# LTLA/batchelor

Hardware: AMD Instinct MI355X
Metric: cells/sec corrected (reducedMNN engine, 50 PCs) (higher is better)
Workload: dtype fp16 MFMA candidate pass (f32 accumulate) + FP64 exact re-rank; 1 GPU; config3: 8 synthetic Gaussian batches x 100000 cells x 50 PCs, k=20, merge.order=1..8, inputs resident in HBM; parallelism=single GPU, exact_fallback_queries=1050

## Files before the change

### batchelor_amd/csrc/abi.hip

```cpp
#include <algorithm>
#include <chrono>
#include <climits>
#include <cstddef>
#include <cmath>
#include <cstdlib>
#include <cstring>
#include <functional>
#include <limits>
#include <memory>
#include <thread>
#include <vector>

#include "bmx_common.hpp"
#include "bmx_ops.hpp"
#include "engine.hpp"
#include "host_xfer.hpp"
#include "mnn_correct.hpp"
#include "rccl_dyn.hpp"
#include "resident_batches.hpp"

struct bmx_engine {
    std::unique_ptr<bmx::Engine> impl;
};
struct bmx_mnn_result {
// ... 140 lines not shown
        }
    });
}

void bmx_trim_caches(void) {
    bmx::DevBlockCache::release_global();
    bmx::StreamPool::release_all();
}

int64_t bmx_last_knn_exact_fallbacks(void) { return g_last_fallbacks; }

void bmx_set_force_exact_knn(int32_t on) { g_force_exact = on; }

int32_t bmx_dev_set(const char* name, int32_t value) {
    if (!name) return BMX_ERR_ARG;
    bmx::DevKnobs& k = bmx::dev_knobs();
    const std::string n(name);
    if (n == "knn_tier") k.knn_tier = value;
    else if (n == "sample") k.sample = value;
    else if (n == "split_c") k.split_c = value;
    else if (n == "force_c") k.force_c = value;
    else if (n == "no_margin") k.no_margin = value;
    else if (n == "asv_fast") k.asv_fast = value;
    else if (n == "asv_cap") k.asv_cap = value;
    else if (n == "sample_split") k.sample_split = value;
    else if (n == "lk_seed") k.lk_seed = value;
    else if (n == "asv_modes") k.asv_modes = value;
    else if (n == "asv_sync") k.asv_sync = value;
    else if (n == "tau_replay") k.tau_replay = value;
    else if (n == "exchange_always") k.exchange_always = value;
    else if (n == "refine_wave") k.refine_wave = value;
    else if (n == "asv_wide") k.asv_wide = value;
    else if (n == "asv_chunk") k.asv_chunk = value;
    else if (n == "reset") k = bmx::DevKnobs();
    else {
        g_last_error = "bmx_dev_set: unknown knob '" + n + "'";
        return BMX_ERR_ARG;
    }
    return BMX_OK;
}

int32_t bmx_dev_get(const char* name, int64_t* value) {
    if (!name || !value) return BMX_ERR_ARG;
    return guarded([&] {
        const std::string n(name);
        unsigned long long t[8];
        if (n == "asv_literal_cells" || n == "asv_fallback_cells" || n == "asv_tiled_cells") {
            bmx::asv_tally_read(t, false);
            *value = (int64_t)t[n == "asv_literal_cells" ? 0 : (n == "asv_fallback_cells" ? 1 : 2)];
        } else if (n == "asv_ticks_stream" || n == "asv_ticks_wait" || n == "asv_ticks_cells") {
            bmx::asv_ticks_read(t);
            *value = (int64_t)t[n == "asv_ticks_stream" ? 0 : (n == "asv_ticks_wait" ? 1 : 2)];
        } else if (n == "asv_ticks_literal" || n == "asv_ticks_chains" || n == "asv_literal_addends" || n == "asv_chain_tiles") {
            bmx::asv_ticks_read(t);
            *value = (int64_t)t[n == "asv_ticks_literal" ? 4 : (n == "asv_ticks_chains" ? 5 : (n == "asv_literal_addends" ? 6 : 7))];
        } else if (n == "delta_gene_tile" || n == "delta_pair_chunk") {
            *value = n == "delta_gene_tile" ? bmx::DELTA_GENE_TILE : bmx::DELTA_PAIR_CHUNK;
        } else if (n == "asv_tally_reset") {
            bmx::asv_tally_read(t, true);
            *value = 0;
        } else {
            throw bmx::Error(BMX_ERR_ARG, "bmx_dev_get: unknown counter '" + n + "'");
        }
    });
}

int32_t bmx_dev_get_bytes(const char* name, void* dst, int64_t n) {
    if (!name || (n > 0 && !dst) || n < 0) return BMX_ERR_ARG;
    return guarded([&] {
        if (std::string(name) != "asv_modes") throw bmx::Error(BMX_ERR_ARG, std::string("bmx_dev_get_bytes: unknown array '") + name + "'");
        bmx::asv_modes_read(static_cast<unsigned char*>(dst), (size_t)n);
    });
}

int32_t bmx_dev_host_copy(void* dst, const void* src, int64_t bytes) {
    if (bytes < 0 || (bytes > 0 && (!dst || !src))) return BMX_ERR_ARG;
    bmx::host_parallel_memcpy(dst, src, (size_t)bytes);
    return BMX_OK;
}

void bmx_shard_range(int64_t n, int32_t rank, int32_t world, int64_t* begin, int64_t* end) {
    bmx::bmx_shard_range_impl(n, rank, world, begin, end);
}

int64_t bmx_shard_gather_bytes(int64_t n, int32_t world, int64_t bytes_per_row) {
    return bmx::bmx_shard_rows_per_rank(n, world) * bytes_per_row;
}

int32_t bmx_query_knn(const double* X, int32_t nx, const double* query, int32_t nq, int32_t d, int32_t k,
                      int32_t* index, double* distance) {
    return guarded([&] {
        if (nx < 0 || nq < 0 || d <= 0 || k < 0) throw bmx::Error(BMX_ERR_ARG, "queryKNN: negative dimension");
        if (k > nx) throw bmx::Error(BMX_ERR_ARG, "queryKNN: 'k' exceeds the number of points in 'X'");
        if (nq == 0 || k == 0) return;
        bmx::Engine& e = prim(d);
        bmx::CacheScope cache_scope(e.cache());
        hipStream_t s = e.stream();
        bmx::DevBuf<double> t1, t2, dX, dQ, dD;
        bmx::DevBuf<int32_t> dI, dIc;
        const double* px = upload_rm(t1, dX, X, nx, d, s);
        const double* pq = upload_rm(t2, dQ, query, nq, d, s);
        int32_t* pi = dI.reserve((size_t)nq * k);
        double* pd = dD.reserve((size_t)nq * k);
        e.knn(px, nullptr, nx, pq, nullptr, nq, k, pi, pd);
        const size_t nres = (size_t)nq * k;
        if (nres >= ((size_t)1 << 22)) {
            g_last_fallbacks = e.knn_ws_.last_exact;
            if (index) {
                int32_t* pc = dIc.reserve(nres);
                hipLaunchKernelGGL(idx_to_r_layout, dim3((unsigned)((nq + 31) / 32), (unsigned)((k + 31) / 32)), dim3(32, 8), 0, s,
                                   (const int32_t*)pi, nq, k, pc);
// ... 678 lines not shown
```

### batchelor_amd/csrc/bmx_common.hpp

```cpp
#pragma once
#include <hip/hip_runtime.h>

#include <atomic>
#include <cstdint>
#include <cstdio>
#include <map>
#include <mutex>
#include <stdexcept>
#include <string>
#include <vector>

#include "../../include/batchelor_mi355x.h"

namespace bmx {

struct Error : std::runtime_error {
    int code;
    Error(int c, const std::string& m) : std::runtime_error(m), code(c) {}
};

#define BMX_HIP(expr)                                                                                   \
    do {                                                                                                \
        hipError_t e_ = (expr);                                                                         \
        if (e_ != hipSuccess)                                                                           \
            throw bmx::Error(BMX_ERR_HIP, std::string(#expr) + " failed: " + hipGetErrorString(e_));    \
    } while (0)

#define BMX_LAUNCH_CHECK() BMX_HIP(hipGetLastError())

struct WatchdogTimeout : Error {
    explicit WatchdogTimeout(const std::string& m) : Error(BMX_ERR_HIP, m) {}
};
void guarded_stream_sync(hipStream_t stream, double budget_s);

#ifndef BMX_KS1
#define BMX_KS1 32
#endif

struct DevKnobs {
    int knn_tier = 0;
    int sample = -1;
    int split_c = 0;
    int force_c = 0;
    int no_margin = 0;
    int asv_fast = 0;
    int asv_cap = -1;
    int asv_modes = 0;
    int asv_sync = 0;
    int tau_replay = 0;
    int lk_seed = 1;
    int sample_split = -1;
    int exchange_always = 0;
    int refine_wave = 0;
    int asv_wide = 0;
    int asv_chunk = 0;
};
DevKnobs& dev_knobs();
bool debug_prints();
bool debug_timings();

inline int cdiv(int64_t a, int64_t b) { return (int)((a + b - 1) / b); }
inline int64_t round_up(int64_t a, int64_t b) { return (a + b - 1) / b * b; }

struct DevBlockCache {
    struct Block {
        void* p;
        size_t bytes;
        int device;
    };
    std::vector<Block> blocks;
    bool leak = false;
    DevBlockCache() = default;
    DevBlockCache(const DevBlockCache&) = delete;
    DevBlockCache& operator=(const DevBlockCache&) = delete;
    struct GlobalPool {
        std::mutex mu;
        std::vector<Block> blocks;
        size_t total = 0;
    };
    static GlobalPool& global() {
        static GlobalPool* g = new GlobalPool();
        return *g;
    }
    ~DevBlockCache() {
        GlobalPool& g = global();
        if (!leak) {
            std::lock_guard<std::mutex> lk(g.mu);
// ... 185 lines not shown
            DevBlockCache* c = DevBlockCache::current();
            if (void* q = c ? c->take(want * sizeof(T), &got) : nullptr) {
                p = static_cast<T*>(q);
                cap = got / sizeof(T);
            } else {
                ++dev_malloc_calls();
                hipError_t e = hipMalloc((void**)&p, want * sizeof(T));
                if (e == hipErrorOutOfMemory) {
                    (void)hipGetLastError();
                    DevBlockCache::release_global();
                    e = hipMalloc((void**)&p, want * sizeof(T));
                }
                if (e != hipSuccess) {
                    p = nullptr;
                    throw bmx::Error(BMX_ERR_HIP, std::string("hipMalloc failed: ") + hipGetErrorString(e));
                }
                cap = want;
            }
        }
        return p;
    }
};

struct KnnWorkspace {
    DevBuf<float> pq, pr;
    DevBuf<double> qn2, rn2, mean, red;
    DevBuf<int32_t> cand;
    DevBuf<float> tau;
    DevBuf<float> cand_v;
    DevBuf<uint32_t> tau_g;
    DevBuf<float> margin;
    std::vector<DevBuf<uint32_t>> tau_rec;
    size_t replay_idx = 0;
    DevBuf<float> samp_lists;
    DevBuf<uint32_t> tau_seed;
    bool slots_clean = false;
    DevBuf<unsigned long long> maxslots;
    DevBuf<int32_t> flagged_t[2], sub_rows[2], sub_idx[2];
    DevBuf<int32_t> lk_rows, lk_idx;
    DevBuf<double> lk_d2;
    bool dist_squared = false;
    DevBuf<double> lk_kth;
    DevBuf<float> lk_seed;
    DevBuf<double> flag_bound_t[2], sub_dist[2];
    DevBuf<double> drow;
    DevBuf<double> xd;
    DevBuf<int32_t> xcnt, xi, slow;
    static constexpr int OPT_CAP = 256;
    bool optimistic = false;
    bool xcnt_clear = false;
    DevBuf<int32_t> opt_state;
    int32_t* opt_state_ptr(hipStream_t s) {
        if (!opt_state.p) {
            opt_state.reserve(8);
            BMX_HIP(hipMemsetAsync(opt_state.p, 0, 8 * sizeof(int32_t), s));
        }
        return opt_state.p;
    }
    int force_exact = 0;
    double wd_budget_s = 0.0;
    void sync(hipStream_t s) const { guarded_stream_sync(s, wd_budget_s); }
    int64_t* pinned_words() {
        if (!pin_) pin_ = static_cast<int64_t*>(pinned_small_take());
        return pin_;
    }
    static constexpr size_t kPinnedSmall = (size_t)64 << 10;
// ... 40 lines not shown
        if (event_tag.size() <= events_used) event_tag.resize(events_used + 1);
        event_tag[events_used] = tag;
        if (events_used == events.size()) {
            hipEvent_t a, b;
            BMX_HIP(hipEventCreate(&a));
            BMX_HIP(hipEventCreate(&b));
            events.emplace_back(a, b);
        }
        return events[events_used++];
    }
    ~KnnWorkspace() {
        if (abandon) return;
        pinned_small_give(pin_);
        for (auto& e : events) {
            (void)hipEventDestroy(e.first);
            (void)hipEventDestroy(e.second);
        }
    }
};

struct Bf16Launch {
    const uint16_t* pq;
    const uint16_t* pr;
    int nqb, first_begin, range_len, nranges, r_limit, out_chunk0, out_nchunks;
    uint32_t* tau_g;
    int sample;
    int32_t* cand;
    float* cand_v;
    float* tau;
    int n_full = 0;
    const float* margin = nullptr;
    int k = 0;
    const uint32_t* tau_seed = nullptr;
};
int bf16_pick_ns(int d);
int bf16_ncons(int NS, int KS);
void bf16_prep(hipStream_t stream, const double* X, const int32_t* rows, int n, int n_pad, int d, int NS,
               const double* mean, int is_query, uint16_t* P, double* n2, unsigned long long* maxbits,
               unsigned long long* slots);
bool bf16_launch(hipStream_t stream, KnnWorkspace& ws, int NS, int KS, const Bf16Launch& L);
int f16_rows_per_slot(int NS, int KS);

void knn_device(hipStream_t stream, KnnWorkspace& ws, const double* X, const int32_t* ref_rows, int nr,
                const double* Q, const int32_t* q_rows, int nq, int d, int k, int32_t* idx_out, double* dist_out,
                int q_begin, int q_end, const float* seed_d2 = nullptr, const double* centre = nullptr,
                double* kth_out = nullptr);

}
```

### batchelor_amd/csrc/knn.hip

```cpp
#include "bmx_common.hpp"
#include "knn_select.hpp"

#include <algorithm>
#include <atomic>
#include <chrono>
#include <cmath>
#include <cstdio>
#include <cstdlib>
#include <thread>

namespace bmx {

int f16_pick_ns(int d, int KS);
void f16_prep_all(hipStream_t stream, const double* X, const int32_t* rrows, int nr, int nr_pad, const double* Q,
                  const int32_t* qrows, int nq, int nq_pad, int d, int NS, const double* mean, uint16_t* Pr, uint16_t* Pq,
                  double* rn2, double* qn2, unsigned long long* maxbits, unsigned long long* slots, int32_t* flagged0,
                  float* margin, const sel::PassEps& pe, const float* seed_d2, uint32_t* tau_seed, uint32_t* tau_init);
bool f16_launch(hipStream_t stream, KnnWorkspace& ws, int NS, int KS, const Bf16Launch& L);
void f16_sample_merge(hipStream_t stream, const float* lists, int nranges, int KS, int nq, int k, const float* margin,
                      uint32_t* tau_g);

namespace {

using namespace sel;

constexpr int MAX_CHUNKS = 8;

__global__ void colsum_partial(const double* __restrict__ X, const int32_t* __restrict__ rows, int n, int d,
                               int rows_per_block, int stride, double* __restrict__ partial) {
    __shared__ double sm[4][64];
    const int c0 = threadIdx.x & 63, rl = threadIdx.x >> 6;
    const int r0 = blockIdx.x * rows_per_block;
    const int r1 = min(n, r0 + rows_per_block);
    for (int cb = 0; cb < d; cb += 64) {
        const int c = cb + c0;
        double s = 0.0;
        if (c < d)
            for (int r = r0 + rl; r < r1; r += 4) {
                const int64_t rs = (int64_t)r * stride;
                const int64_t row = rows ? rows[rs] : rs;
                s += X[row * d + c];
            }
        sm[rl][c0] = s;
        __syncthreads();
        if (rl == 0 && c < d) partial[(int64_t)blockIdx.x * d + c] = (sm[0][c0] + sm[1][c0]) + (sm[2][c0] + sm[3][c0]);
        __syncthreads();
    }
}

__global__ void colsum_final(const double* __restrict__ partial, int nblocks, int d, double scale,
                             double* __restrict__ out) {
    const int c = blockIdx.x * blockDim.x + threadIdx.x;
    if (c >= d) return;
    double s = 0.0;
    for (int b = 0; b < nblocks; ++b) s += partial[(int64_t)b * d + c];
    out[c] = s * scale;
}


// ... 841 lines not shown

int candidate_tiers(int d, int k, int nr, Tier out[2]) {
    const int only = dev_knobs().knn_tier;
    int n = 0;
    if (k > 36) return 0;
    const int KS1 = k <= 20 ? BMX_KS1 : 48, KS2 = k <= 20 ? 24 : 40;
    const int ns1 = f16_pick_ns(d, KS1);
    if (ns1 && nr > 2 * KS1 && (only == 0 || only == 1)) out[n++] = Tier{1, ns1, KS1};
    const int ns2 = bf16_pick_ns(d);
    if (ns2 && !(KS2 == 40 && ns2 > 16) && nr > 2 * KS2 && (only == 0 || only == 2)) out[n++] = Tier{2, ns2, KS2};
    return n;
}

void candidate_pass(hipStream_t stream, KnnWorkspace& ws, const Tier& T, const double* X, const int32_t* ref_rows, int nr,
                    const double* Qs, const int32_t* qrs, int nq, int d, int k, int32_t* io, double* dout,
                    int32_t* flagged, double* flag_bound, const float* seed_d2, const double* centre, double* kth_out) {
    const int NS = T.NS, KS = T.KS;
    ws.last_variant = T.id == 1 ? 3 : 2;
    const int unit = T.id == 1 ? 256 : 32 * bf16_ncons(NS, KS);
    const int nq_pad = (int)round_up(nq, unit);
    const int nqb = nq_pad / unit;

    const bool no_margin_knob = dev_knobs().no_margin != 0;
    int S_auto = nr >= 32768 ? 4096 : 0;
    if (T.id == 1 && nr >= 4096) S_auto = std::max(1024, std::min(nr / 4, NS <= 4 ? 24576 : 12288));
    if (seed_d2 && T.id == 1) S_auto = std::min(S_auto, BMX_SEEDED_SAMPLE);
    int S = (int)round_up(dev_knobs().sample >= 0 ? dev_knobs().sample : S_auto, T.id == 1 ? f16_rows_per_slot(NS, KS) : 64);
    int CS = 1;
    if (T.id == 1 && S > 0 && nqb < 128 && dev_knobs().sample_split != 0 && !no_margin_knob) {
        const int rs = f16_rows_per_slot(NS, KS);
        CS = std::max(1, std::min({256 / std::max(nqb, 1), 8, S / (8 * rs)}));
        if (dev_knobs().sample_split > 0) CS = std::max(1, std::min({dev_knobs().sample_split, S / rs, 512 / KS}));
    }
    int C = 1, n_full = 0;
    {
        const int a = nqb / 256, b = nqb % 256;
        n_full = a * 256;
        if (b > 0) {
            double best = 1e30;
            for (int c = 1; c <= MAX_CHUNKS - 1; ++c) {
                if (c > 1 && nr / c < 2048) break;
                const double tailc = std::ceil((double)b * c / 256.0) / c * (1.0 + 0.105 * std::log((double)c));
                if (tailc < best - 1e-9) {
                    best = tailc;
                    C = c;
                }
            }
        }
    }
    if (dev_knobs().split_c > 0) C = std::max(1, dev_knobs().split_c);
    if (dev_knobs().force_c > 0) {
        C = std::max(1, std::min(MAX_CHUNKS - 1, dev_knobs().force_c));
        n_full = 0;
    }
    const int rmul = T.id == 1 ? f16_rows_per_slot(NS, KS) : 32;
    const int chunk_len = (int)round_up(cdiv(nr, C), rmul);
    C = std::max(1, cdiv(nr, chunk_len));
    const int nr_pad = chunk_len * C;
    const int nchunks = C;
    S = std::min(S, nr_pad / rmul * rmul);
    if (debug_prints())
        fprintf(stderr, "[bmx] knn tier %d: nq=%d nr=%d d=%d NS=%d KS=%d S=%d C=%d chunk=%d full-range blocks=%d of %d\n", T.id,
                nq, nr, d, NS, KS, S, C, chunk_len, C > 1 ? n_full : nqb, nqb);

    const int KPw = 8 * NS;
    float* pq = ws.pq.reserve((size_t)nq_pad * KPw);
    float* pr = ws.pr.reserve((size_t)(nr_pad + 256) * KPw);
    double* qn2 = ws.qn2.reserve(nq_pad);
    double* rn2 = ws.rn2.reserve(nr_pad);
    double* mean = ws.mean.reserve((size_t)d + 2);
    unsigned long long* maxbits = reinterpret_cast<unsigned long long*>(mean + d);
    int32_t* cand = ws.cand.reserve((size_t)nq_pad * nchunks * KS);
    float* cand_v = ws.cand_v.reserve((size_t)nq_pad * nchunks * KS);
    float* tau = ws.tau.reserve((size_t)nq_pad * nchunks);
    uint32_t* tau_g = ws.tau_g.reserve(nq_pad);
    unsigned long long* slots = ws.maxslots.reserve(64 * 16);

    if (!centre) {
        const int cstride = std::max(1, nr / 16384);
        const int ncs = cdiv(nr, cstride);
        const int rpb = 256;
        const int nb = cdiv(ncs, rpb);
        double* red = ws.red.reserve((size_t)nb * d);
        hipLaunchKernelGGL(colsum_partial, dim3(nb), dim3(256), 0, stream, X, ref_rows, ncs, d, rpb, cstride, red);
        BMX_LAUNCH_CHECK();
        hipLaunchKernelGGL(colsum_final, dim3(cdiv(d, 64)), dim3(64), 0, stream, red, nb, d, 1.0 / ncs, mean);
        BMX_LAUNCH_CHECK();
        centre = mean;
    }
    PassEps pe;
    if (T.id == 1) {
        pe.eps_k = 16.0 * NS;
        pe.eps_qr = 2.0;
        pe.eps_split = 2.0 * (0.0009765625 + 2.384185791015625e-07);
        pe.eps_den = 6.103515625e-05 * (std::sqrt((double)d) + 3.0);
        pe.scaled = 1;
// ... 35 lines not shown
                L.nranges = cdiv(S, L.range_len);
                if (L.nranges > 1 && margin) {
                    lists = ws.samp_lists.reserve((size_t)nq_pad * L.nranges * KS);
                    L.cand_v = lists;
                }
            }
            ok = go(L);
            if (lists) f16_sample_merge(stream, lists, L.nranges, KS, nq, k, margin, tau_g);
            L.cand_v = cand_v;
        }
    } else {
        ws.slots_clean = false;
        BMX_HIP(hipMemsetAsync(maxbits, 0, sizeof(unsigned long long), stream));
        bf16_prep(stream, X, ref_rows, nr, nr_pad, d, NS, centre, 0, reinterpret_cast<uint16_t*>(pr), rn2, maxbits, slots);
        bf16_prep(stream, Qs, qrs, nq, nq_pad, d, NS, centre, 1, reinterpret_cast<uint16_t*>(pq), qn2, maxbits, slots);
        if (S == 0) {
            hipLaunchKernelGGL(fill_u32, dim3(cdiv(nq_pad, 256)), dim3(256), 0, stream, tau_g, nq_pad, 0xFF800000u);
            BMX_LAUNCH_CHECK();
        }
        if (S > 0) ok = go(L);
        if (seed_d2) {
            hipLaunchKernelGGL(seed_tau_kernel, dim3(cdiv(nq_pad, 256)), dim3(256), 0, stream, seed_d2, qn2, maxbits, nq, nq_pad,
                               pe, tau_g);
            BMX_LAUNCH_CHECK();
        }
        BMX_HIP(hipMemsetAsync(flagged, 0, sizeof(int32_t), stream));
    }
    L.first_begin = 0;
    L.range_len = chunk_len;
    L.nranges = C;
    L.n_full = C > 1 ? n_full : 0;
    L.r_limit = nr_pad;
    L.sample = 0;
    const int replay = T.id == 1 ? dev_knobs().tau_replay : 0;
    if (replay == 2 && ws.replay_idx < ws.tau_rec.size() && ws.tau_rec[ws.replay_idx].cap >= (size_t)nq_pad) {
        hipLaunchKernelGGL(tau_apply_kernel, dim3(cdiv(nq_pad, 256)), dim3(256), 0, stream,
                           (const uint32_t*)ws.tau_rec[ws.replay_idx].p, nq_pad, tau_g);
        BMX_LAUNCH_CHECK();
    }
    ok = ok && go(L);
    if (replay == 1) {
        if (ws.tau_rec.size() <= ws.replay_idx) ws.tau_rec.resize(ws.replay_idx + 1);
        hipLaunchKernelGGL(tau_record_kernel, dim3(cdiv(nq_pad, 256)), dim3(256), 0, stream, (const float*)tau, nchunks, nq_pad,
                           ws.tau_rec[ws.replay_idx].reserve((size_t)nq_pad));
        BMX_LAUNCH_CHECK();
    }
    if (replay) ++ws.replay_idx;
    if (!ok) throw Error(BMX_ERR_ARG, "kNN: unsupported padded dimension");
    {
        const int need = (d & 1) ? 0 : cdiv(d, 8);
        const int unit_q = T.id == 1 ? 256 : 32 * bf16_ncons(NS, KS);
        const int nq_half = KS == 32 && !dev_knobs().refine_wave ? (C > 1 ? std::min(nq, n_full * unit_q) : nq) : 0;
        const int sq = ws.dist_squared ? 1 : 0;
#define BMX_REFINE(NC)                                                                                                              \
    do {                                                                                                                            \
        if (nq_half > 0)                                                                                                            \
            hipLaunchKernelGGL(knn_refine_half<NC>, dim3(cdiv(nq_half, 8)), dim3(256), 0, stream, X, ref_rows, Qs, qrs, nq_half, d, k, \
                               nchunks, eps_k, eps_qr, eps_split, eps_den, T.id == 1 ? 1 : 0, cand, cand_v, tau, qn2, maxbits,       \
                               seed_d2, io, dout, flagged, flag_bound, zero_slots, kth_out, sq);                                    \
        if (nq > nq_half)                                                                                                           \
            hipLaunchKernelGGL(knn_refine<NC>, dim3(cdiv(nq - nq_half, 4)), dim3(256), 0, stream, X, ref_rows, Qs, qrs, nq, d, k, KS,  \
                               nchunks, eps_k, eps_qr, eps_split, eps_den, T.id == 1 ? 1 : 0, cand, cand_v, tau, qn2, maxbits,       \
                               seed_d2, io, dout, flagged, flag_bound, nq_half > 0 ? nullptr : zero_slots, nq_half, kth_out, sq);   \
    } while (0)
        if (need == 0 || need > 16) BMX_REFINE(0);
        else if (need <= 2) BMX_REFINE(2);
        else if (need <= 4) BMX_REFINE(4);
        else if (need <= 7) BMX_REFINE(7);
        else if (need <= 10) BMX_REFINE(10);
        else if (need <= 13) BMX_REFINE(13);
        else BMX_REFINE(16);
#undef BMX_REFINE
    }
    BMX_LAUNCH_CHECK();
    if (zero_slots) ws.slots_clean = true;
    if (debug_prints()) {
        std::vector<int32_t> hc((size_t)nq * nchunks * KS);
        BMX_HIP(hipMemcpyAsync(hc.data(), cand, hc.size() * sizeof(int32_t), hipMemcpyDeviceToHost, stream));
        ws.sync(stream);
        size_t valid = 0;
        for (int32_t v : hc) valid += v >= 0;
        fprintf(stderr, "[bmx] candidates per query after the top-k pass: %.1f (of %d slots)\n", (double)valid / nq,
                nchunks * KS);
    }
}
// ... 671 lines not shown
```

### batchelor_amd/csrc/knn_f16.hip

```cpp
#include "bmx_common.hpp"
#include "knn_select.hpp"

#include <cmath>
#include <string>

namespace bmx {
namespace {

using namespace sel;
typedef _Float16 f16x8 __attribute__((ext_vector_type(8)));

constexpr int NCONS = 8;
constexpr int NPROD = 2;
#ifndef BMX_NSERV
#define BMX_NSERV 4
#endif
__host__ __device__ constexpr int serv_waves(int NS) { return NS <= 5 ? BMX_NSERV : 2; }
constexpr int NQ = NCONS * 32;
constexpr int QCAP = 64;
#ifndef BMX_DRAIN_MIN
#define BMX_DRAIN_MIN 16
#endif
#ifndef BMX_SPRIO
#define BMX_SPRIO 0
// ... 209 lines not shown
#ifndef BMX_LCAP_MAX
#define BMX_LCAP_MAX 56
#endif
#ifndef BMX_TP_MAX
#define BMX_TP_MAX 2
#endif
__host__ __device__ constexpr int tile_pairs_for(int NS, int KS) {
    return (BMX_TP_MAX >= 2 && KS + 16 <= BMX_LCAP_MAX && ring_slots_for(NS, KS + 16, 2) >= 3) ? 2 : 1;
}
__host__ __device__ constexpr int list_cap(int NS, int KS) {
    const int TP = tile_pairs_for(NS, KS);
    for (int c = BMX_LCAP_MAX; c >= KS + 16; c -= 8)
        if (ring_slots_for(NS, c, TP) >= (TP == 2 ? 3 : 2)) return c;
    return KS + 16 <= 64 ? KS + 16 : 64;
}

__device__ __forceinline__ int lds_load_volatile(const int* p) {
    return __hip_atomic_load(p, __ATOMIC_RELAXED, __HIP_MEMORY_SCOPE_WORKGROUP);
}
__device__ __forceinline__ int mbcnt64(unsigned long long m) {
    return __builtin_amdgcn_mbcnt_hi((uint32_t)(m >> 32), __builtin_amdgcn_mbcnt_lo((uint32_t)m, 0u));
}

#ifdef BMX_STAMPS
__device__ unsigned long long bmx_dbg16[48];
#define STAMP() __builtin_readcyclecounter()
#endif

template <int NS, int KS, int LCAP, bool SAMPLE>
__global__ __launch_bounds__((NCONS + NPROD + serv_waves(NS)) * 64) void knn_topk_f16(
    const uint16_t* __restrict__ Pq, const uint16_t* __restrict__ PrF, int first_begin, int range_len, int r_limit,
    int n_full, int nranges, int out_chunk0, int out_nchunks, uint32_t* __restrict__ tau_g, int32_t* __restrict__ cand,
    float* __restrict__ cand_v, float* __restrict__ tau_out, const float* __restrict__ margin_g, int kq,
    const uint32_t* __restrict__ tau_seed) {
    constexpr int TILE_BYTES = NS * 1024;
    constexpr int TP = tile_pairs_for(NS, KS);
    constexpr int SLOT_BYTES = TP * 2 * TILE_BYTES;
    constexpr int NSLOT = ring_slots_for(NS, LCAP, TP);
    static_assert(NSLOT >= 2, "LDS ring");
    static_assert(LCAP <= 64 && LCAP > KS, "one list entry per lane during compaction");
    constexpr int KEEP_MAX = KS + 11 < LCAP - 4 ? KS + 11 : LCAP - 4;
    static_assert(KEEP_MAX >= KS, "list capacity");
    constexpr int NSERV = serv_waves(NS);
    static_assert(NCONS % NSERV == 0 && (NCONS / NSERV) % 2 == 0, "a service wave's consumers: whole groups of 64 queries");
    static_assert((QCAP & (QCAP - 1)) == 0 && QCAP >= 64, "queue positions wrap by masking; one group can hold 64 records");

    extern __shared__ __attribute__((aligned(16))) char smem[];
    char* ring = smem;
    unsigned long long* lists = reinterpret_cast<unsigned long long*>(smem + NSLOT * SLOT_BYTES);
    float* qvals = reinterpret_cast<float*>(lists + NQ * LCAP);
    uint32_t* qtags = reinterpret_cast<uint32_t*>(qvals + NCONS * QCAP * 4);
    int* cnt = reinterpret_cast<int*>(qtags + NCONS * QCAP);
    float* tauL = reinterpret_cast<float*>(cnt + NQ);
    float* mgL = tauL + NQ;
    int* ready = reinterpret_cast<int*>(mgL + NQ);
    int* done = ready + NSLOT;
    int* wrL = done + NSLOT;
    int* rdL = wrL + NCONS;
    int* stL = rdL + NCONS;
#ifdef BMX_EXP_ROWFILTER
    float* rtau = reinterpret_cast<float*>(stL + NCONS);
    if (threadIdx.x < 32) rtau[threadIdx.x] = -__builtin_inff();
#endif

    const int tid = threadIdx.x, lane = tid & 63;
    const int wave = __builtin_amdgcn_readfirstlane(tid >> 6);
    int qblock = blockIdx.x, rng = 0, nrng = 1, r_begin = first_begin, r_end = r_limit;
    if ((int)blockIdx.x >= n_full) {
        const int nsplit = (gridDim.x - n_full) / nranges, jx = blockIdx.x - n_full;
        rng = jx / nsplit;
        qblock = n_full + (jx - rng * nsplit);
        nrng = nranges;
        r_begin = first_begin + rng * range_len;
        r_end = min(r_limit, r_begin + range_len);
    }
    const int ntiles = (r_end - r_begin) >> 5;
    const int nslots = ntiles / (2 * TP);
    const int out_chunk = out_chunk0 + rng;
    if (tid < 2 * NSLOT + 3 * NCONS) ready[tid] = 0;
    if (tid < NQ) {
        cnt[tid] = 0;
        tauL[tid] = (!SAMPLE && tau_g) ? orderable_f32(tau_g[qblock * NQ + tid]) : __builtin_inff();
        mgL[tid] = (!SAMPLE && margin_g) ? margin_g[qblock * NQ + tid] : 0.f;
    }
    __syncthreads();
    const bool shared_tau = !SAMPLE && tau_g != nullptr && nrng > 1;

#ifdef BMX_STAMPS
    unsigned long long dbg_ncomp = 0, dbg_comp = 0, dbg_rounds = 0;
#endif
    auto compact = [&](const int c, const int jj, const bool exact) __attribute__((always_inline)) {
        unsigned long long* mylists = lists + c * 32 * LCAP;
        int* mycnt = cnt + c * 32;
        const int n_raw = __builtin_amdgcn_readfirstlane(lds_load_volatile(&mycnt[jj]));
        const int n = n_raw < LCAP ? n_raw : LCAP;
        if (n <= KS && (n < kq || margin_g == nullptr)) return;
#ifdef BMX_STAMPS
        const unsigned long long c0 = STAMP();
        ++dbg_ncomp;
#endif
        const unsigned long long raw = lane < n ? mylists[jj * LCAP + lane] : 0ull;
// ... 72 lines not shown
        const int pos = mbcnt64(keep);
        __builtin_amdgcn_fence(__ATOMIC_ACQ_REL, "wavefront");
        if ((keep >> lane) & 1ull) mylists[jj * LCAP + pos] = raw;
        if (lane == 0) mycnt[jj] = nkeep;
        if (lane == jj) {
            const float told = tauL[c * 32 + jj];
            tauL[c * 32 + jj] = newtau < told ? newtau : told;
            if (shared_tau) atomicMin(&tau_g[qblock * NQ + c * 32 + jj], f32_orderable(newtau));
        }
        __builtin_amdgcn_fence(__ATOMIC_ACQ_REL, "wavefront");
#ifdef BMX_STAMPS
        dbg_comp += STAMP() - c0;
#endif
    };

    auto out_lists = [&](const int c, const int j0, const int j1) __attribute__((always_inline)) {
        unsigned long long* mylists = lists + c * 32 * LCAP;
        int* mycnt = cnt + c * 32;
        for (int jj = j0; jj < j1; ++jj) compact(c, jj, true);
        for (int jj = j0; jj < j1; ++jj) {
            const int qq = qblock * NQ + c * 32 + jj;
            const int n = __builtin_amdgcn_readfirstlane(lds_load_volatile(&mycnt[jj]));
            const float eff = __uint_as_float((uint32_t)__builtin_amdgcn_readfirstlane(
                (int)__float_as_uint(__hip_atomic_load(&tauL[c * 32 + jj], __ATOMIC_RELAXED, __HIP_MEMORY_SCOPE_WORKGROUP))));
            if (lane < KS) {
                const unsigned long long e = lane < n ? mylists[jj * LCAP + lane] : 0ull;
                const float val = __uint_as_float((uint32_t)(e >> 32));
                const bool keep = lane < n && (val < eff || nrng == 1);
                const int64_t o = ((int64_t)qq * out_nchunks + out_chunk) * KS + lane;
                cand[o] = keep ? (int32_t)(uint32_t)e : -1;
                cand_v[o] = lane < n ? val : __builtin_inff();
            }
            if (lane == 0) tau_out[(int64_t)qq * out_nchunks + out_chunk] = eff;
            if (nrng == 1) {
                for (int cc = 1; cc < out_nchunks; ++cc) {
                    if (lane < KS) cand[((int64_t)qq * out_nchunks + out_chunk + cc) * KS + lane] = -1;
                    if (lane == 0) tau_out[(int64_t)qq * out_nchunks + out_chunk + cc] = __builtin_inff();
                }
            }
        }
    };

    if (wave >= NCONS && wave < NCONS + NPROD) {
#ifdef BMX_EXP_PPRIO
        __builtin_amdgcn_s_setprio(BMX_EXP_PPRIO);
#endif
        const int p = wave - NCONS;
        f32x4 ra[2 * NS], rb[2 * NS];
        const f32x4* src = reinterpret_cast<const f32x4*>(PrF) + ((int64_t)(r_begin >> 5) * NS) * 64 + lane;
        f32x4* ring_l = reinterpret_cast<f32x4*>(ring) + lane;
        auto load = [&](f32x4(&r)[2 * NS], int sl) {
#pragma unroll
            for (int s = 0; s < 2 * NS; ++s) r[s] = src[((int64_t)sl * 2 * NS + s) * 64];
        };
        auto wait_free = [&](int sl, int pos) __attribute__((always_inline)) {
            if (sl < NSLOT) return;
            const int need = (sl / NSLOT) * NCONS;
            while (__builtin_amdgcn_readfirstlane(lds_load_volatile(&done[pos])) < need)
                __builtin_amdgcn_s_sleep(BMX_PSLEEP);
        };
        auto publish = [&](const f32x4(&r)[2 * NS], int sl) {
            const int pos = sl % NSLOT;
            wait_free(sl, pos);
            __atomic_signal_fence(__ATOMIC_SEQ_CST);
            f32x4* dst = ring_l + pos * (SLOT_BYTES / 16);
#pragma unroll
            for (int s = 0; s < 2 * NS; ++s) dst[s * 64] = r[s];
            __atomic_signal_fence(__ATOMIC_SEQ_CST);
            if (lane == 0) __hip_atomic_store(&ready[pos], sl + 1, __ATOMIC_RELAXED, __HIP_MEMORY_SCOPE_WORKGROUP);
        };
// ... 527 lines not shown
        out_lists(wave, 0, EPI_CONS);
#ifdef BMX_STAMPS
        if (lane == 0) {
            atomicAdd(&bmx_dbg16[0], STAMP() - dbg_t0);
            atomicAdd(&bmx_dbg16[1], dbg_spin);
            atomicAdd(&bmx_dbg16[6], dbg_evt);
            atomicAdd(&bmx_dbg16[7], dbg_grp);
            atomicAdd(&bmx_dbg16[8], (unsigned long long)ntiles);
            atomicAdd(&bmx_dbg16[9], 1ull);
            atomicAdd(&bmx_dbg16[10], dbg_evc);
            atomicAdd(&bmx_dbg16[12], dbg_qwait);
        }
#endif
    }
}

template <int NS, int KS>
void launch(hipStream_t stream, KnnWorkspace& ws, const Bf16Launch& L) {
    constexpr int LCAP = list_cap(NS, KS);
    constexpr int TP = tile_pairs_for(NS, KS);
    constexpr size_t lds =
        (size_t)ring_slots_for(NS, LCAP, TP) * TP * 2 * NS * 1024 + (size_t)NQ * LCAP * 8 + lds_fixed_bytes();
    static_assert(lds <= 160 * 1024, "LDS budget");
    ensure_dynamic_lds(reinterpret_cast<const void*>(&knn_topk_f16<NS, KS, LCAP, false>), lds);
    ensure_dynamic_lds(reinterpret_cast<const void*>(&knn_topk_f16<NS, KS, LCAP, true>), lds);
    std::pair<hipEvent_t, hipEvent_t> ev{nullptr, nullptr};
    if (ws.profile) {
        ev = ws.next_events(L.sample ? 0 : 1);
        BMX_HIP(hipEventRecord(ev.first, stream));
    }
    if (!L.sample)
        ws.last_kernel = "knn_topk_f16<" + std::to_string(NS) + ", " + std::to_string(KS) + ", " + std::to_string(LCAP) +
                         ", false>";
    const int items = L.n_full + (L.nqb - L.n_full) * L.nranges;
    if (L.sample)
        hipLaunchKernelGGL((knn_topk_f16<NS, KS, LCAP, true>), dim3(items), dim3((NCONS + NPROD + serv_waves(NS)) * 64), lds, stream,
                           L.pq, L.pr, L.first_begin, L.range_len, L.r_limit, L.n_full, L.nranges, L.out_chunk0,
                           L.out_nchunks, L.tau_g, L.cand, L.cand_v, L.tau, L.margin, L.k, L.tau_seed);
    else
        hipLaunchKernelGGL((knn_topk_f16<NS, KS, LCAP, false>), dim3(items), dim3((NCONS + NPROD + serv_waves(NS)) * 64), lds, stream,
                           L.pq, L.pr, L.first_begin, L.range_len, L.r_limit, L.n_full, L.nranges, L.out_chunk0,
                           L.out_nchunks, L.tau_g, L.cand, L.cand_v, L.tau, L.margin, L.k, (const uint32_t*)nullptr);
    BMX_LAUNCH_CHECK();
    if (ws.profile) BMX_HIP(hipEventRecord(ev.second, stream));
#ifdef BMX_STAMPS
    {
        if (L.sample) fprintf(stderr, "(sample pass) ");
        unsigned long long hh[48];
        BMX_HIP(hipStreamSynchronize(stream));
        BMX_HIP(hipMemcpyFromSymbol(hh, HIP_SYMBOL(bmx_dbg16), sizeof(hh)));
        const double nt = (double)hh[8];
        const double sw = hh[14] ? (double)hh[14] : 1.0;
        fprintf(stderr,
                "[stamps f16] consumers=%.0f tiles/wave=%.0f cyc/tile=%.0f spin/tile=%.0f evpath/tile=%.0f qwait/tile=%.0f "
                "event tiles=%.3f groups/tile=%.3f | service waves=%.0f cyc=%.0f drain=%.0f (%.0f passes, %.0f cyc each) "
                "compact=%.0f (%.0f calls, %.1f rounds each) idle polls=%.0f\n",
                (double)hh[9], nt / hh[9], hh[0] / nt, hh[1] / nt, hh[10] / nt, hh[12] / nt, hh[6] / nt, hh[7] / nt,
                (double)hh[14], hh[13] / sw, hh[2] / sw, hh[3] / sw, hh[3] ? (double)hh[2] / hh[3] : 0.0, hh[5] / sw,
                hh[4] / sw, hh[4] ? (double)hh[11] / hh[4] : 0.0, hh[15] / sw);
        unsigned long long z[48] = {0};
        BMX_HIP(hipMemcpyToSymbol(HIP_SYMBOL(bmx_dbg16), z, sizeof(z)));
    }
#endif
}

}

namespace {
__global__ __launch_bounds__(256) void sample_merge_kernel(const float* __restrict__ lists, int n, int len, int nq, int k,
                                                           const float* __restrict__ margin_g, uint32_t* __restrict__ tau_g) {
    (void)len;
    const int w = threadIdx.x >> 6, lane = threadIdx.x & 63;
    const int q = blockIdx.x * 4 + w;
    if (q >= nq) return;
    uint32_t val[8];
// ... 79 lines not shown
```

### include/batchelor_mi355x.h

```cpp
#ifndef BATCHELOR_MI355X_H
#define BATCHELOR_MI355X_H

#include <stdint.h>

#ifdef __cplusplus
extern "C" {
#endif

#define BMX_OK 0
#define BMX_ERR_HIP (-1)
#define BMX_ERR_DIM_GENES (-2)
#define BMX_ERR_DIM_CELLS (-3)
#define BMX_ERR_SUBSET (-4)
#define BMX_ERR_INDEX_LEN (-5)
#define BMX_ERR_ARG (-6)
#define BMX_ERR_TREE (-7)
#define BMX_ERR_NO_PAIRS (-8)
#define BMX_ERR_EXCHANGE (-9)

const char* bmx_last_error(void);
int32_t bmx_device_count(void);
void bmx_free(void* p);
int32_t bmx_set_device(int32_t device);
void bmx_trim_caches(void);


int32_t bmx_find_mutual_nns(const int32_t* left, int32_t nL, int32_t k2, const int32_t* right, int32_t nR, int32_t k1,
                            int32_t** out_left, int32_t** out_right, int64_t* npairs);

int32_t bmx_smooth_gaussian_kernel(const double* averaged, int32_t g, int32_t U, const int32_t* index,
                                   int32_t index_len, const double* mat, int32_t gd, int32_t n, double sigma2,
                                   double* out);

int32_t bmx_adjust_shift_variance(const double* data1, int32_t g1, int32_t n1, const double* data2, int32_t g2,
                                  int32_t n2, const double* vect, int32_t vrow, int32_t vcol, double sigma2,
                                  const int32_t* restrict1, int32_t nr1, const int32_t* restrict2, int32_t nr2,
                                  double* out);

int32_t bmx_adjust_shift_variance_form(int32_t n2, int32_t nr1, int32_t nr2);


int32_t bmx_query_knn(const double* X, int32_t nx, const double* query, int32_t nq, int32_t d, int32_t k,
                      int32_t* index, double* distance);

int32_t bmx_find_mutual_nn(const double* data1, int32_t n1, const double* data2, int32_t n2, int32_t d, int32_t k1,
                           int32_t k2, int32_t** first, int32_t** second, int64_t* npairs);

int64_t bmx_last_knn_exact_fallbacks(void);
void bmx_set_force_exact_knn(int32_t on);
int32_t bmx_dev_set(const char* name, int32_t value);
int32_t bmx_dev_get(const char* name, int64_t* value);
int32_t bmx_dev_get_bytes(const char* name, void* dst, int64_t n);
double bmx_last_native_kernel_ms(void);
int32_t bmx_dev_host_copy(void* dst, const void* src, int64_t bytes);

typedef struct bmx_engine bmx_engine_t;

typedef struct {
    int32_t struct_size;
    int32_t k;
    double prop_k;
    double ndist;
    double min_batch_skip;
    int32_t auto_merge;
    int32_t var_adj;
    double sigma;
} bmx_params_t;

typedef int32_t (*bmx_allgather_fn)(void* ctx, void* buf, int64_t bytes_per_rank);

int32_t bmx_engine_create(int32_t device, bmx_engine_t** out);
void bmx_engine_destroy(bmx_engine_t* e);
int32_t bmx_engine_set_shard(bmx_engine_t* e, int32_t rank, int32_t world, bmx_allgather_fn fn, void* ctx);
int32_t bmx_rccl_load(const char* librccl_path);
int32_t bmx_rccl_unique_id(void* id_out, int32_t bytes);
int32_t bmx_engine_init_rccl(bmx_engine_t* e, int32_t rank, int32_t world, const void* unique_id, int32_t bytes);
int32_t bmx_engine_exchange_stats(bmx_engine_t* e, int64_t* calls, int64_t* bytes);
int32_t bmx_engine_upload(bmx_engine_t* e, int32_t nbatches, int32_t d, const double* const* data,
                          const int32_t* nrows, const int32_t* const* restrict_idx, const int32_t* n_restrict);
int32_t bmx_engine_run(bmx_engine_t* e, const bmx_params_t* params, const int32_t* tree, int32_t tree_len);
int32_t bmx_engine_download(bmx_engine_t* e, double* corrected, int32_t* batch, int32_t* merge_left,
                            int32_t* merge_right, double* batch_size, int32_t* skipped, double* lost_var);
int32_t bmx_engine_pairs(bmx_engine_t* e, int32_t merge, int32_t** left, int32_t** right, int64_t* npairs);
int32_t bmx_engine_pairs_into(bmx_engine_t* e, int32_t merge, int32_t* left, int32_t* right, int64_t capacity,
                              int64_t* npairs);
int32_t bmx_engine_pairs_all_into(bmx_engine_t* e, int32_t nmerges, int32_t* const* left, int32_t* const* right,
                                  const int64_t* capacity);
// ... 144 lines not shown
```

Measured before the change: 9.444 million cells/s.

## Balance kNN tail work with explicit per-block work-item table

Replaces the uniform chunk split of leftover query blocks (beyond full CU waves) with a host-built plan. The plan cuts the tail's reference ranges into near-equal pieces across CUs and picks the lowest simulated makespan, falling back to the uniform split when that is cheaper. The f16 kernel now reads its qblock, range and output chunk from a device item table, which is cached per shape. This aims to cut idle CUs in the last wave, at the cost of more uneven per-query segment counts, a table read per block, and changed padding of nr.

```diff
diff --git a/batchelor_amd/csrc/abi.hip b/batchelor_amd/csrc/abi.hip
--- a/batchelor_amd/csrc/abi.hip
+++ b/batchelor_amd/csrc/abi.hip
@@ -196,6 +196,8 @@
     else if (n == "refine_wave") k.refine_wave = value;
     else if (n == "asv_wide") k.asv_wide = value;
     else if (n == "asv_chunk") k.asv_chunk = value;
+    else if (n == "plan_cus") k.plan_cus = value;
+    else if (n == "plan_uniform") k.plan_uniform = value;
     else if (n == "reset") k = bmx::DevKnobs();
     else {
         g_last_error = "bmx_dev_set: unknown knob '" + n + "'";
@@ -241,6 +243,21 @@
     if (bytes < 0 || (bytes > 0 && (!dst || !src))) return BMX_ERR_ARG;
     bmx::host_parallel_memcpy(dst, src, (size_t)bytes);
     return BMX_OK;
+}
+
+int32_t bmx_dev_knn_plan(int32_t nqb, int32_t nr, int32_t rmul, int32_t cus, int32_t split_c, int32_t force_c,
+                         int32_t plan_uniform, int32_t* items, int32_t cap, int32_t* info, double* costs) {
+    if (nqb < 1 || nr < 1 || rmul < 1 || cus < 1 || cap < 0 || (cap > 0 && !items) || !info || !costs) return BMX_ERR_ARG;
+    const bmx::KnnPlan pl =
+        bmx::plan_knn_items(nqb, nr, rmul, cus, bmx::KNN_MAX_CHUNKS, split_c, force_c, plan_uniform != 0);
+    static_assert(sizeof(bmx::KnnItem) == 5 * sizeof(int32_t), "five words an item");
+    std::memcpy(items, pl.items.data(), std::min((size_t)cap, pl.items.size()) * sizeof(bmx::KnnItem));
+    const int32_t inf[8] = {pl.n_full, pl.nchunks, pl.nr_pad, pl.balanced, pl.pieces, pl.seg_min, pl.seg_max,
+                            bmx::KNN_MAX_CHUNKS - 1};
+    std::memcpy(info, inf, sizeof(inf));
+    costs[0] = pl.cost_uniform;
+    costs[1] = pl.cost_balanced;
+    return (int32_t)pl.items.size();
 }
 
 void bmx_shard_range(int64_t n, int32_t rank, int32_t world, int64_t* begin, int64_t* end) {
diff --git a/batchelor_amd/csrc/bmx_common.hpp b/batchelor_amd/csrc/bmx_common.hpp
--- a/batchelor_amd/csrc/bmx_common.hpp
+++ b/batchelor_amd/csrc/bmx_common.hpp
@@ -1,6 +1,7 @@
 #pragma once
 #include <hip/hip_runtime.h>
 
+#include <array>
 #include <atomic>
 #include <cstdint>
 #include <cstdio>
@@ -11,6 +12,7 @@
 #include <vector>
 
 #include "../../include/batchelor_mi355x.h"
+#include "knn_plan.hpp"
 
 namespace bmx {
 
@@ -53,6 +55,8 @@
     int exchange_always = 0;
     int refine_wave = 0;
     int asv_wide = 0;
+    int plan_cus = 0;
+    int plan_uniform = 0;
     int asv_chunk = 0;
 };
 DevKnobs& dev_knobs();
@@ -304,6 +308,7 @@
     DevBuf<float> margin;
     std::vector<DevBuf<uint32_t>> tau_rec;
     size_t replay_idx = 0;
+    std::map<std::array<int, 7>, DevBuf<int32_t>> plan_tabs;
     DevBuf<float> samp_lists;
     DevBuf<uint32_t> tau_seed;
     bool slots_clean = false;
@@ -410,6 +415,8 @@
     const float* margin = nullptr;
     int k = 0;
     const uint32_t* tau_seed = nullptr;
+    const KnnItem* items = nullptr;
+    int nitems = 0;
 };
 int bf16_pick_ns(int d);
 int bf16_ncons(int NS, int KS);
diff --git a/batchelor_amd/csrc/knn.hip b/batchelor_amd/csrc/knn.hip
--- a/batchelor_amd/csrc/knn.hip
+++ b/batchelor_amd/csrc/knn.hip
@@ -24,7 +24,7 @@
 
 using namespace sel;
 
-constexpr int MAX_CHUNKS = 8;
+constexpr int MAX_CHUNKS = KNN_MAX_CHUNKS;
 
 __global__ void colsum_partial(const double* __restrict__ X, const int32_t* __restrict__ rows, int n, int d,
                                int rows_per_block, int stride, double* __restrict__ partial) {
@@ -932,36 +932,22 @@
         CS = std::max(1, std::min({256 / std::max(nqb, 1), 8, S / (8 * rs)}));
         if (dev_knobs().sample_split > 0) CS = std::max(1, std::min({dev_knobs().sample_split, S / rs, 512 / KS}));
     }
-    int C = 1, n_full = 0;
-    {
-        const int a = nqb / 256, b = nqb % 256;
-        n_full = a * 256;
-        if (b > 0) {
-            double best = 1e30;
-            for (int c = 1; c <= MAX_CHUNKS - 1; ++c) {
-                if (c > 1 && nr / c < 2048) break;
-                const double tailc = std::ceil((double)b * c / 256.0) / c * (1.0 + 0.105 * std::log((double)c));
-                if (tailc < best - 1e-9) {
-                    best = tailc;
-                    C = c;
-                }
-            }
-        }
-    }
-    if (dev_knobs().split_c > 0) C = std::max(1, dev_knobs().split_c);
-    if (dev_knobs().force_c > 0) {
-        C = std::max(1, std::min(MAX_CHUNKS - 1, dev_knobs().force_c));
-        n_full = 0;
-    }
     const int rmul = T.id == 1 ? f16_rows_per_slot(NS, KS) : 32;
-    const int chunk_len = (int)round_up(cdiv(nr, C), rmul);
-    C = std::max(1, cdiv(nr, chunk_len));
-    const int nr_pad = chunk_len * C;
-    const int nchunks = C;
+    const int plan_cus = dev_knobs().plan_cus > 0 ? dev_knobs().plan_cus : PLAN_CUS;
+    const bool plan_uniform = T.id != 1 || dev_knobs().plan_uniform != 0;
+    const KnnPlan plan =
+        plan_knn_items(nqb, nr, rmul, plan_cus, MAX_CHUNKS, dev_knobs().split_c, dev_knobs().force_c, plan_uniform);
+    const int C = plan.uniform_c, chunk_len = plan.uniform_len;
+    const int n_full = plan.n_full;
+    const int nr_pad = plan.nr_pad;
+    const int nchunks = plan.nchunks;
     S = std::min(S, nr_pad / rmul * rmul);
     if (debug_prints())
-        fprintf(stderr, "[bmx] knn tier %d: nq=%d nr=%d d=%d NS=%d KS=%d S=%d C=%d chunk=%d full-range blocks=%d of %d\n", T.id,
-                nq, nr, d, NS, KS, S, C, chunk_len, C > 1 ? n_full : nqb, nqb);
+        fprintf(stderr,
+                "[bmx] knn tier %d: nq=%d nr=%d d=%d NS=%d KS=%d S=%d plan=%s items=%d pieces=%d segments/block=%d..%d "
+                "full-range blocks=%d of %d tail cost: uniform(C=%d, chunk=%d) %.3f balanced %.3f sweeps\n",
+                T.id, nq, nr, d, NS, KS, S, plan.balanced ? "balanced" : "uniform", (int)plan.items.size(), plan.pieces,
+                plan.seg_min, plan.seg_max, n_full, nqb, C, chunk_len, plan.cost_uniform, plan.cost_balanced);
 
     const int KPw = 8 * NS;
     float* pq = ws.pq.reserve((size_t)nq_pad * KPw);
@@ -1063,6 +1049,19 @@
     L.n_full = C > 1 ? n_full : 0;
     L.r_limit = nr_pad;
     L.sample = 0;
+    if (T.id == 1) {
+        const std::array<int, 7> key{nqb, nr, rmul, plan_cus, dev_knobs().split_c, dev_knobs().force_c, plan_uniform ? 1 : 0};
+        auto tab = ws.plan_tabs.find(key);
+        if (tab == ws.plan_tabs.end()) {
+            if (ws.plan_tabs.size() >= 256) ws.plan_tabs.clear();
+            tab = ws.plan_tabs.emplace(key, DevBuf<int32_t>()).first;
+            const size_t words = plan.items.size() * (sizeof(KnnItem) / sizeof(int32_t));
+            BMX_HIP(hipMemcpyAsync(tab->second.reserve(words), plan.items.data(), words * sizeof(int32_t), hipMemcpyHostToDevice,
+                                   stream));
+        }
+        L.items = reinterpret_cast<const KnnItem*>(tab->second.p);
+        L.nitems = (int)plan.items.size();
+    }
     const int replay = T.id == 1 ? dev_knobs().tau_replay : 0;
     if (replay == 2 && ws.replay_idx < ws.tau_rec.size() && ws.tau_rec[ws.replay_idx].cap >= (size_t)nq_pad) {
         hipLaunchKernelGGL(tau_apply_kernel, dim3(cdiv(nq_pad, 256)), dim3(256), 0, stream,
@@ -1081,7 +1080,7 @@
     {
         const int need = (d & 1) ? 0 : cdiv(d, 8);
         const int unit_q = T.id == 1 ? 256 : 32 * bf16_ncons(NS, KS);
-        const int nq_half = KS == 32 && !dev_knobs().refine_wave ? (C > 1 ? std::min(nq, n_full * unit_q) : nq) : 0;
+        const int nq_half = KS == 32 && !dev_knobs().refine_wave ? std::min<int64_t>(nq, (int64_t)n_full * unit_q) : 0;
         const int sq = ws.dist_squared ? 1 : 0;
 #define BMX_REFINE(NC)                                                                                                              \
     do {                                                                                                                            \
diff --git a/batchelor_amd/csrc/knn_f16.hip b/batchelor_amd/csrc/knn_f16.hip
--- a/batchelor_amd/csrc/knn_f16.hip
+++ b/batchelor_amd/csrc/knn_f16.hip
@@ -265,7 +265,7 @@
     const uint16_t* __restrict__ Pq, const uint16_t* __restrict__ PrF, int first_begin, int range_len, int r_limit,
     int n_full, int nranges, int out_chunk0, int out_nchunks, uint32_t* __restrict__ tau_g, int32_t* __restrict__ cand,
     float* __restrict__ cand_v, float* __restrict__ tau_out, const float* __restrict__ margin_g, int kq,
-    const uint32_t* __restrict__ tau_seed) {
+    const uint32_t* __restrict__ tau_seed, const KnnItem* __restrict__ items) {
     constexpr int TILE_BYTES = NS * 1024;
     constexpr int TP = tile_pairs_for(NS, KS);
     constexpr int SLOT_BYTES = TP * 2 * TILE_BYTES;
@@ -299,7 +299,14 @@
     const int tid = threadIdx.x, lane = tid & 63;
     const int wave = __builtin_amdgcn_readfirstlane(tid >> 6);
     int qblock = blockIdx.x, rng = 0, nrng = 1, r_begin = first_begin, r_end = r_limit;
-    if ((int)blockIdx.x >= n_full) {
+    if constexpr (!SAMPLE) {
+        const KnnItem it = items[blockIdx.x];
+        qblock = it.qblock;
+        r_begin = it.r_begin;
+        r_end = it.r_end;
+        rng = it.out_chunk;
+        nrng = it.split;
+    } else if ((int)blockIdx.x >= n_full) {
         const int nsplit = (gridDim.x - n_full) / nranges, jx = blockIdx.x - n_full;
         rng = jx / nsplit;
         qblock = n_full + (jx - rng * nsplit);
@@ -438,10 +445,10 @@
                 cand_v[o] = lane < n ? val : __builtin_inff();
             }
             if (lane == 0) tau_out[(int64_t)qq * out_nchunks + out_chunk] = eff;
-            if (nrng == 1) {
-                for (int cc = 1; cc < out_nchunks; ++cc) {
-                    if (lane < KS) cand[((int64_t)qq * out_nchunks + out_chunk + cc) * KS + lane] = -1;
-                    if (lane == 0) tau_out[(int64_t)qq * out_nchunks + out_chunk + cc] = __builtin_inff();
+            if (rng == nrng - 1) {
+                for (int cc = out_chunk + 1; cc < out_chunk0 + out_nchunks; ++cc) {
+                    if (lane < KS) cand[((int64_t)qq * out_nchunks + cc) * KS + lane] = -1;
+                    if (lane == 0) tau_out[(int64_t)qq * out_nchunks + cc] = __builtin_inff();
                 }
             }
         }
@@ -1035,15 +1042,16 @@
     if (!L.sample)
         ws.last_kernel = "knn_topk_f16<" + std::to_string(NS) + ", " + std::to_string(KS) + ", " + std::to_string(LCAP) +
                          ", false>";
-    const int items = L.n_full + (L.nqb - L.n_full) * L.nranges;
+    if (!L.sample && (!L.items || L.nitems < 1)) throw Error(BMX_ERR_ARG, "kNN: a full pass without its work items");
     if (L.sample)
-        hipLaunchKernelGGL((knn_topk_f16<NS, KS, LCAP, true>), dim3(items), dim3((NCONS + NPROD + serv_waves(NS)) * 64), lds, stream,
-                           L.pq, L.pr, L.first_begin, L.range_len, L.r_limit, L.n_full, L.nranges, L.out_chunk0,
-                           L.out_nchunks, L.tau_g, L.cand, L.cand_v, L.tau, L.margin, L.k, L.tau_seed);
+        hipLaunchKernelGGL((knn_topk_f16<NS, KS, LCAP, true>), dim3(L.n_full + (L.nqb - L.n_full) * L.nranges),
+                           dim3((NCONS + NPROD + serv_waves(NS)) * 64), lds, stream, L.pq, L.pr, L.first_begin, L.range_len,
+                           L.r_limit, L.n_full, L.nranges, L.out_chunk0, L.out_nchunks, L.tau_g, L.cand, L.cand_v, L.tau,
+                           L.margin, L.k, L.tau_seed, (const KnnItem*)nullptr);
     else
-        hipLaunchKernelGGL((knn_topk_f16<NS, KS, LCAP, false>), dim3(items), dim3((NCONS + NPROD + serv_waves(NS)) * 64), lds, stream,
-                           L.pq, L.pr, L.first_begin, L.range_len, L.r_limit, L.n_full, L.nranges, L.out_chunk0,
-                           L.out_nchunks, L.tau_g, L.cand, L.cand_v, L.tau, L.margin, L.k, (const uint32_t*)nullptr);
+        hipLaunchKernelGGL((knn_topk_f16<NS, KS, LCAP, false>), dim3(L.nitems), dim3((NCONS + NPROD + serv_waves(NS)) * 64), lds,
+                           stream, L.pq, L.pr, L.first_begin, L.range_len, L.r_limit, L.n_full, L.nranges, L.out_chunk0,
+                           L.out_nchunks, L.tau_g, L.cand, L.cand_v, L.tau, L.margin, L.k, (const uint32_t*)nullptr, L.items);
     BMX_LAUNCH_CHECK();
     if (ws.profile) BMX_HIP(hipEventRecord(ev.second, stream));
 #ifdef BMX_STAMPS
diff --git a/batchelor_amd/csrc/knn_plan.hpp b/batchelor_amd/csrc/knn_plan.hpp
--- /dev/null
+++ b/batchelor_amd/csrc/knn_plan.hpp
@@ -0,0 +1,158 @@
+#pragma once
+#include <algorithm>
+#include <cmath>
+#include <cstdint>
+#include <functional>
+#include <queue>
+#include <vector>
+
+namespace bmx {
+
+constexpr int KNN_MAX_CHUNKS = 8;
+constexpr int PLAN_CUS = 256;
+constexpr int PLAN_MIN_SEG_ROWS = 2048;
+constexpr double PLAN_SPLIT_LN = 0.105;
+
+struct KnnItem {
+    int32_t qblock;
+    int32_t r_begin, r_end;
+    int32_t out_chunk;
+    int32_t split;
+};
+
+struct KnnPlan {
+    std::vector<KnnItem> items;
+    int n_full = 0;
+    int nchunks = 1;
+    int nr_pad = 0;
+    int balanced = 0;
+    int uniform_c = 1, uniform_len = 0;
+    int pieces = 0;
+    int seg_min = 1, seg_max = 1;
+    double cost_uniform = 0.0, cost_balanced = -1.0;
+};
+
+inline double plan_penalty(int s) { return 1.0 + PLAN_SPLIT_LN * std::log((double)std::max(1, s)); }
+
+inline double plan_makespan(const std::vector<KnnItem>& items, size_t first, int nr_pad, int cus) {
+    std::priority_queue<double, std::vector<double>, std::greater<double>> free_at;
+    for (int i = 0; i < cus; ++i) free_at.push(0.0);
+    double span = 0.0;
+    for (size_t i = first; i < items.size(); ++i) {
+        const double t = free_at.top() + (double)(items[i].r_end - items[i].r_begin) / nr_pad * plan_penalty(items[i].split);
+        free_at.pop();
+        free_at.push(t);
+        span = std::max(span, t);
+    }
+    return span;
+}
+
+inline bool plan_balanced_tail(int n_full, int nqb, int nr_pad, int rmul, int P, int max_seg, std::vector<KnnItem>& out) {
+    const int64_t T = nr_pad / rmul;
+    const int64_t b = nqb - n_full, W = b * T;
+    const int64_t min_u = (PLAN_MIN_SEG_ROWS + rmul - 1) / rmul;
+    std::vector<int64_t> cuts;
+    int64_t j = 1;
+    for (int64_t i = 0; i < b; ++i) {
+        const int64_t lo = i * T, hi = lo + T;
+        cuts.clear();
+        int64_t last = lo;
+        for (;; ++j) {
+            const int64_t c = (2 * j * W + P) / (2 * (int64_t)P);
+            if (j >= P || c >= hi) break;
+            if (c - last >= min_u) {
+                cuts.push_back(c);
+                last = c;
+            }
+        }
+        if (!cuts.empty() && hi - cuts.back() < min_u) cuts.pop_back();
+        const int s = (int)cuts.size() + 1;
+        if (s > max_seg) return false;
+        int64_t from = lo;
+        for (int c = 0; c < s; ++c) {
+            const int64_t to = c + 1 < s ? cuts[c] : hi;
+            out.push_back(KnnItem{(int32_t)(n_full + i), (int32_t)((from - lo) * rmul), (int32_t)((to - lo) * rmul), c, s});
+            from = to;
+        }
+    }
+    return true;
+}
+
+inline KnnPlan plan_knn_items(int nqb, int nr, int rmul, int cus, int max_chunks, int split_c = 0, int force_c = 0,
+                              bool no_balance = false) {
+    KnnPlan pl;
+    cus = std::max(1, cus);
+    const int a = nqb / cus, b = nqb % cus;
+    int n_full = a * cus, C = 1;
+    if (b > 0) {
+        double best = 1e30;
+        for (int c = 1; c <= max_chunks - 1; ++c) {
+            if (c > 1 && nr / c < PLAN_MIN_SEG_ROWS) break;
+            const double tailc = std::ceil((double)b * c / cus) / c * plan_penalty(c);
+            if (tailc < best - 1e-9) {
+                best = tailc;
+                C = c;
+            }
+        }
+    }
+    const bool forced = split_c > 0 || force_c > 0;
+    if (split_c > 0) C = std::max(1, split_c);
+    if (force_c > 0) {
+        C = std::max(1, std::min(max_chunks - 1, force_c));
+        n_full = 0;
+    }
+    const int64_t chunk_len = (((int64_t)nr + C - 1) / C + rmul - 1) / rmul * rmul;
+    C = std::max(1, (int)((nr + chunk_len - 1) / chunk_len));
+    pl.uniform_c = C;
+    pl.uniform_len = (int)chunk_len;
+    pl.cost_uniform = b > 0 || force_c > 0 ? std::ceil((double)(nqb - n_full) * C / cus) / C * plan_penalty(C) : 0.0;
+
+    std::vector<KnnItem> tail, cand;
+    const int nr_bal = (int)(((int64_t)nr + rmul - 1) / rmul * rmul);
+    if (b > 0 && !forced && !no_balance) {
+        for (int m = 1; m <= 3; ++m) {
+            cand.clear();
+            if (!plan_balanced_tail(n_full, nqb, nr_bal, rmul, m * cus, max_chunks - 1, cand)) break;
+            int most = 1;
+            for (const KnnItem& it : cand) most = std::max(most, (int)it.split);
+            if (most > C) break;
+            std::stable_sort(cand.begin(), cand.end(), [](const KnnItem& x, const KnnItem& y) {
+                return x.r_end - x.r_begin > y.r_end - y.r_begin;
+            });
+            const double cost = plan_makespan(cand, 0, nr_bal, cus);
+            if (pl.cost_balanced < 0.0 || cost < pl.cost_balanced - 1e-9) {
+                pl.cost_balanced = cost;
+                pl.pieces = m * cus;
+                tail.swap(cand);
+            }
+        }
+    }
+    pl.balanced = pl.cost_balanced >= 0.0 && pl.cost_balanced < pl.cost_uniform - 1e-9 ? 1 : 0;
+    if (pl.balanced) {
+        pl.nr_pad = nr_bal;
+        pl.n_full = n_full;
+        for (int qb = 0; qb < n_full; ++qb) pl.items.push_back(KnnItem{qb, 0, pl.nr_pad, 0, 1});
+        pl.items.insert(pl.items.end(), tail.begin(), tail.end());
+        pl.seg_min = max_chunks;
+        pl.seg_max = 1;
+        for (const KnnItem& it : tail) {
+            pl.seg_min = std::min(pl.seg_min, (int)it.split);
+            pl.seg_max = std::max(pl.seg_max, (int)it.split);
+        }
+        pl.nchunks = pl.seg_max;
+    } else {
+        pl.nr_pad = (int)(chunk_len * C);
+        pl.n_full = C > 1 ? n_full : nqb;
+        pl.nchunks = C;
+        pl.seg_min = pl.seg_max = C;
+        pl.pieces = 0;
+        for (int qb = 0; qb < pl.n_full; ++qb) pl.items.push_back(KnnItem{qb, 0, pl.nr_pad, 0, 1});
+        for (int rng = 0; rng < C && pl.n_full < nqb; ++rng)
+            for (int qb = pl.n_full; qb < nqb; ++qb)
+                pl.items.push_back(KnnItem{qb, (int32_t)(rng * chunk_len),
+                                           (int32_t)std::min<int64_t>(pl.nr_pad, (rng + 1) * chunk_len), rng, C});
+    }
+    return pl;
+}
+
+}
diff --git a/include/batchelor_mi355x.h b/include/batchelor_mi355x.h
--- a/include/batchelor_mi355x.h
+++ b/include/batchelor_mi355x.h
@@ -53,6 +53,8 @@
 int32_t bmx_dev_get_bytes(const char* name, void* dst, int64_t n);
 double bmx_last_native_kernel_ms(void);
 int32_t bmx_dev_host_copy(void* dst, const void* src, int64_t bytes);
+int32_t bmx_dev_knn_plan(int32_t nqb, int32_t nr, int32_t rmul, int32_t cus, int32_t split_c, int32_t force_c,
+                         int32_t plan_uniform, int32_t* items, int32_t cap, int32_t* info, double* costs);
 
 typedef struct bmx_engine bmx_engine_t;
 
```

Result: no change. 9.524 million cells/s, median of 6 (+0.9%).
